# JiaxuanYou/graph-pooling

Measured on AMD Instinct MI355X. Metric: graphs/sec fwd+bwd, DD padded batch N_max=500, higher is better.
Workload: dtype f32; 1 GPU; S-DD: DD-shaped padded batch, B=20/GPU, N_max=500, F=89, H=E=20, K=50, L=3, 1 pool; graphs_per_gpu=20, global_batch=20, linkpred=False, hip_graph=True, parallelism=dp1

## Files before the change

graph_pooling_amd/csrc/dp_common.h:

```cpp
#pragma once
#include <hip/hip_runtime.h>
#include <cstddef>
#include <cstdint>
#include <cstdio>
#include <cstring>
#include <atomic>
#include <mutex>

#include "../../include/diffpool_hip.h"

namespace dp {

void set_error(const char* fmt, ...);
const char* last_error();

#define DP_CHECK_ARG(cond, ...)                      \
    do {                                             \
        if (!(cond)) {                               \
            ::dp::set_error(__VA_ARGS__);            \
            return DP_ERR_INVALID_ARG;               \
        }                                            \
    } while (0)

int* device_error_word();
// ... 449 lines not shown
    const float* stats[DP_MAX_LAYERS];
    const float* Z[2];
    int ldz[2];
    int coff[2][DP_MAX_LAYERS];
    int K;
    long wp_off, bp_off;
    const float* S;
    const float* Tt;
    const float* dXn;
    const float* dAn;
    const float* d_assign;
    const float* dZe;
    const unsigned short *pkA, *pkAt;
    int pk_ld;
    const int* pk_flag;
    const int* pk_sym;
    float* slabs;
    long slab_gstride;
    unsigned short* vs;
    float* part;
    float* gpart;
    int* bar;
};
bool level0_bwd_persistent_ok(const Level0Bwd& a);
size_t level0_bwd_vs_elems(const Level0Bwd& a);
size_t level0_bwd_gpart_floats(const Level0Bwd& a);
void level0_backward(Seq& q, const Level0Bwd& a);
bool level0_persistent_ok(const Level0Fwd& a);
size_t level0_bar_ints(int B);
int* level0_seq_word(int* bar);
size_t level0_xpart_floats(const Level0Fwd& a);
size_t level0_vs_elems(const Level0Fwd& a);
size_t level0_part_floats(const Level0Fwd& a);
size_t level0_mpart_floats(const Level0Fwd& a);
const int* level0_error_word(const int* bar);
void level0_forward(Seq& q, const Level0Fwd& a);

struct HeadArgs {
    const float* Z;
    int ldz, n, rw, featoff;
    int* argmax;
    int lda;
    const float* params;
    int n_pred;
    int dims[DP_MAX_PRED + 2];
    long w_off[DP_MAX_PRED + 1], b_off[DP_MAX_PRED + 1];
    float* hid[DP_MAX_PRED + 2];
    int B;
    long long* labels;
    const int* poison[DP_MAX_LEVELS + 1];
    int n_poison;
};
struct HeadBwdArgs {
    HeadArgs h;
    const float* d_ypred;
    float* grads;
    int n_levels;
    struct Level {
        float* dZ;
        const int* argmax;
        int lda, n, ldz, rw, featoff;
    } lv[DP_MAX_LEVELS + 1];
};
bool head_supported(const HeadArgs& a);
void head_fwd(Seq& q, const HeadArgs& a);
void head_bwd(Seq& q, const HeadBwdArgs& a);

bool small_level_fused_ok(int B, int n, const int* dims, int L, bool dadj);
size_t small_level_part_floats(int B, int n, int L);
void small_level_fwd(Seq& q, const SmallLevelIO& io, int B, int n, const int* dims, int L, int add_self, int bn);
struct SmallHeadFold {
    HeadBwdArgs hb;
    int level;
    int zcol;
    float* part;
};
size_t small_head_fold_part_floats(const HeadArgs& h);
long head_grad_entries(const HeadArgs& h);
void reduce_slabs_head(Seq& q, const float* slabs, long stride, int B, float* out, long count,
                       const SmallHeadFold& hf);
bool small_head_fold_fits(int B, int n, const int* dims, int L, bool dadj, const HeadArgs& h);
void small_level_bwd(Seq& q, const SmallLevelIO& io, const float* dZe, float* dX0, float* dadj, float* slabs,
                     long slab_stride, int B, int n, const int* dims, int L, int add_self, int bn,
                     const SmallHeadFold* hf = nullptr);

void build_batch(Seq& q, const int* src, const int* dst, const int* edge_ptr, const int* label, const int* node_ptr,
                 float* adj, unsigned short* pk, unsigned short* pkt, float* feats, float* assign, int* num_nodes,
                 int* errors, int* degree, int B, int N, int F, int mode, int symmetric, int max_edges_per_graph);

void gather_labels(Seq& q, const long long* src, long long* dst, int B);

void clip_adam_step(Seq& q, float* params, float* grads, float* exp_avg, float* exp_avg_sq, long n, float max_norm,
                    float beta1, float beta2, float eps, float step_size, float inv_bc2_sqrt, float* total_norm_out,
                    int* step_counter = nullptr, float lr = 0.f);

void csr_aggregate_fwd(Seq& q, const float* table, int ldt, const int* indptr, const int* indices, float* out, int ldo,
                       int n_rows, int feat, int mean, float beta, const float* values = nullptr);
void csr_aggregate_bwd_scatter(Seq& q, const float* dout, int ldo, const int* indptr, const int* indices, float* dtable,
                               int ldt, int n_rows, int feat, int mean, const float* values = nullptr);

void segment_max_part(Seq& q, const float* Z, int ldz, const int* chunk_tab, int n_chunks, int F, float* pv, int* pi);

void set2set_prep_weights(Seq& q, const float* w_ih, const float* w_hh, float* wt, int d);

struct LinkPlan {
    int kt, cw;
    int col_tiles, splits, split_tiles;
    int fwd_tiles;
    size_t fwd_lds, bwd_lds;
};
bool linkpred_plan(int B, int n, int K, LinkPlan& p);
void linkpred_fwd(Seq& q, const float* S, int lds, const float* adj, const int* num_nodes, float* loss_out,
                  int B, int n, int K, const float* norm = nullptr );
void linkpred_bwd(Seq& q, const float* S, int lds, const float* adj, const int* num_nodes, const float* dloss,
                  float* dS, int ldds, int B, int n, int K, int accumulate, const float* norm = nullptr);
void linkpred_fwd_packed(Seq& q, const float* S, int lds, const unsigned short* pk, const int* num_nodes,
                         float* loss_out, int B, int n, int K, const float* norm = nullptr);
void linkpred_bwd_packed(Seq& q, const float* S, int lds, const unsigned short* pk, const unsigned short* pkt,
                         const int* num_nodes, const float* dloss, float* dS, int ldds, int B, int n, int K,
                         int accumulate, const float* norm = nullptr);

struct AssignEntPick {
    int lanes;
    int quad;
};
AssignEntPick assign_ent_pick(const void* S, int lds, const void* dS, int ldds, int K);
size_t assign_ent_part_doubles();
void assign_entropy_fwd(Seq& q, const float* S, int lds, const int* num_nodes, float weight, float* ent_out,
                        float* total_inout, int B, int n, int K);
void assign_entropy_bwd(Seq& q, const float* S, int lds, const int* num_nodes, const float* dloss, float weight,
                        float* dS, int ldds, int accumulate, int B, int n, int K);

size_t frob_link_ws_doubles(long long rows, int B, int K);
void frob_link_w_dense(Seq& q, const float* S, int lds, const void* adj, const void* adj_t, int packed, int ld,
                       const int* num_nodes, float* W, int B, int N, int K);
void frob_link_fwd(Seq& q, const float* S, int lds, const float* W, const void* adj, int adj_kind, int adj_ld,
                   const int* num_nodes, const int* node_off, const int* nnz_ptr, const float* link_norm, float wscale,
                   float* G, float* loss_out, float* total_inout, int B, int N, long long rows, int K,
                   const int* csr_indptr = nullptr );
void frob_link_bwd(Seq& q, const float* S, int lds, const float* W, const float* G, const int* num_nodes,
                   const int* node_off, const float* link_norm, const float* dloss, float wscale, float* dS, int ldds,
                   int accumulate, int B, int N, long long rows, int K);

}
```

graph_pooling_amd/csrc/dp_level0.hip:

```cpp
#include "dp_common.h"
#include <type_traits>
#include <utility>
#include <vector>

namespace dp {

#ifdef DP_STAMP
__device__ unsigned long long g_l0_stamps[3][64];
#define L0_STAMP(i)                                                                                    \
    do {                                                                                               \
        if (threadIdx.x == 0 && (wid == 0 || wid == (int)gridDim.x / 2 || wid == (int)gridDim.x - 1)) \
            g_l0_stamps[wid == 0 ? 0 : (wid == (int)gridDim.x - 1 ? 2 : 1)][i] = __builtin_amdgcn_s_memtime(); \
    } while (0)
#else
#define L0_STAMP(i) \
    do {            \
    } while (0)
#endif

namespace {

typedef float f32x4 __attribute__((ext_vector_type(4)));
typedef float f32x4_u __attribute__((ext_vector_type(4), aligned(4)));
typedef short s16x8 __attribute__((ext_vector_type(8)));
// ... 111 lines not shown
        int* pollw = a.f.bar + BAR_GRAPH0 + b * BAR_GSTRIDE;
        const int target = ep.graph * a.T + a.target_bias;
        if (ok) {
            int it = 0;
            while (ag_ld(pollw) < target) {
                if (++it > a.spin_limit) {
                    ok = 0;
                    ag_st(a.f.bar + BAR_ERR, 1);
                    dev_err_raise(a.dev_err, DP_DEVERR_BARRIER);
                    break;
                }
                __builtin_amdgcn_s_sleep(1);
            }
        }
        sflag[0] = ok;
        if (!ok) sflag[1] = 1;
    }
    __syncthreads();
    return sflag[0] != 0;
}
template <typename Args>
__device__ inline bool l0_barrier(const Args& a, int b, int* sflag, L0Epoch& ep) {
    l0_arrive(a, b, sflag, ep);
    return l0_wait(a, b, sflag, ep);
}

template <int NI, typename Args>
__device__ __forceinline__ bool l0_poll_entries(const Args& a, ScBuf buf, const unsigned (&off)[NI], int B, unsigned tag,
                                                float (&v0)[NI][L0_BPAIRS], float (&v1)[NI][L0_BPAIRS], int* sflag) {
    const int tl = threadIdx.x & 15;
    const unsigned want = tag ^ (a.target_bias ? 0x40000000u : 0u);
    int it = 0;
    for (;;) {
        bool ready = true;
#pragma unroll
        for (int j = 0; j < NI; ++j) {
#pragma unroll
            for (int u = 0; u < L0_BPAIRS; ++u) {
                if (16 * u < B) {
                    const u32x4 q = sc_ld16(buf, off[j] + 16u * (unsigned)min(tl + 16 * u, B - 1));
                    v0[j][u] = __uint_as_float(q[0]);
                    v1[j][u] = __uint_as_float(q[2]);
                    ready = ready && q[1] == want && q[3] == want;
                } else {
                    v0[j][u] = 0.f;
                    v1[j][u] = 0.f;
                }
            }
        }
        if (__all(ready)) return true;
        if (++it > a.spin_limit || sflag[1]) {
            if (!sflag[1]) {
                sflag[1] = 1;
                ag_st(a.f.bar + BAR_ERR, 1);
                dev_err_raise(a.dev_err, DP_DEVERR_BARRIER);
            }
            return false;
        }
        __builtin_amdgcn_s_sleep(2);
    }
}

template <int QN>
__device__ __forceinline__ void l0_copy_in(float* dst, const float* src, int count, int zero_to = 0) {
    const int nq = count >> 2;
    float tail = 0.f;
    const int te = (nq << 2) + (int)threadIdx.x;
    if (te < count) tail = src[te];
    for (int base = 0; base < nq; base += QN * L0_NT) {
        f32x4_u q[QN];
#pragma unroll
        for (int u = 0; u < QN; ++u)
            q[u] = *reinterpret_cast<const f32x4_u*>(src + 4 * min(base + u * L0_NT + (int)threadIdx.x, nq - 1));
#pragma unroll
        for (int u = 0; u < QN; ++u) {
            const int e4 = base + u * L0_NT + (int)threadIdx.x;
            if (e4 < nq) *reinterpret_cast<f32x4*>(dst + 4 * e4) = q[u];
        }
    }
    if (te < count) dst[te] = tail;
    for (int e = count + (int)threadIdx.x; e < zero_to; e += L0_NT) dst[e] = 0.f;
}

template <int QN>
struct L0CopyStage {
    f32x4_u q[QN];
    float tail;
};
template <int QN>
__device__ __forceinline__ void l0_copy_issue(L0CopyStage<QN>& s, const float* src, int count, const void* safe) {
    const int nq = count >> 2;
    s.tail = src[min((nq << 2) + (int)threadIdx.x, count - 1)];
    const float* const qs = nq > 0 ? src : static_cast<const float*>(safe);
#pragma unroll
    for (int u = 0; u < QN; ++u)
        s.q[u] = *reinterpret_cast<const f32x4_u*>(qs + 4 * min(u * L0_NT + (int)threadIdx.x, max(nq - 1, 0)));
}
template <int QN>
__device__ __forceinline__ void l0_copy_commit(const L0CopyStage<QN>& s, float* dst, int count, int zero_to = 0) {
    const int nq = count >> 2;
    const int te = (nq << 2) + (int)threadIdx.x;
#pragma unroll
    for (int u = 0; u < QN; ++u) {
        const int e4 = u * L0_NT + (int)threadIdx.x;
        if (e4 < nq) *reinterpret_cast<f32x4*>(dst + 4 * e4) = s.q[u];
    }
    if (te < count) dst[te] = s.tail;
    for (int e = count + (int)threadIdx.x; e < zero_to; e += L0_NT) dst[e] = 0.f;
}
template <int QN>
__device__ __forceinline__ void l0_copy_rest(float* dst, const float* src, int count) {
    const int nq = count >> 2;
#pragma unroll 1
    for (int e4 = QN * L0_NT + (int)threadIdx.x; e4 < nq; e4 += L0_NT)
        *reinterpret_cast<f32x4*>(dst + 4 * e4) = *reinterpret_cast<const f32x4_u*>(src + 4 * e4);
}

__device__ inline void l0_write_split(ScBuf vsb, const float* PT, int ct, int CTt, int K8, int k8_0, int nk8, int nrows) {
    const long pl = (long)CTt * K8 * 128;
    const int items = nk8 * CTt * 16;
    for (int item = threadIdx.x; item < items; item += L0_NT) {
        const int c = item & 15, t = item >> 4;
        const int k8l = t / CTt, cb = t - k8l * CTt;
        const int vc = cb * 16 + c, lr = k8l * 8;
        u16x8 h, m, l;
#pragma unroll
        for (int j = 0; j < 8; ++j) {
            const float v = (vc < ct && lr + j < nrows) ? PT[(lr + j) * ct + min(vc, ct - 1)] : 0.f;
            unsigned short hh, mm, ll;
            bf16_split3(v, hh, mm, ll);
            h[j] = hh; m[j] = mm; l[j] = ll;
        }
        const long o = vs_index(0, CTt, K8, cb, k8_0 + k8l, c, 0);
        sc_st16(vsb, (unsigned)(o * 2), __builtin_bit_cast(u32x4, h));
        sc_st16(vsb, (unsigned)((o + pl) * 2), __builtin_bit_cast(u32x4, m));
        sc_st16(vsb, (unsigned)((o + 2 * pl) * 2), __builtin_bit_cast(u32x4, l));
    }
}

template <int MI, int CTH>
__device__ __forceinline__ void l0_agg_bf16(const unsigned short* Alds, int ldp, const unsigned short* vsp, int CTt, int K8,
                                            int steps, int rot, int cb0, f32x4 (&acc)[MI][CTH]) {
    int lane = threadIdx.x & 63;
    asm volatile("" : "+v"(lane));
    const int kh = __builtin_amdgcn_readfirstlane(threadIdx.x >> 6) & 3;
    const int l15 = lane & 15, kq = lane >> 4;
    auto eff = [&](int step) {
        const int s2 = min(step, steps - 1) + rot;
        return s2 >= steps ? s2 - steps : s2;
    };
    auto load_b = [&](int step, s16x8 (&dst)[3][CTH]) {
        const int st = eff(step);
#pragma unroll
        for (int p = 0; p < 3; ++p)
#pragma unroll
            for (int cbi = 0; cbi < CTH; ++cbi) {
                const int cb = min(cb0 + cbi, CTt - 1);
                const long o = ((((long)p * CTt + cb) * K8 + st * 4 + kq) * 16 + l15) * 8;
                dst[p][cbi] = *reinterpret_cast<const s16x8*>(vsp + o);
            }
    };
    auto mma = [&](int step, const s16x8 (&bf)[3][CTH]) {
        s16x8 av[MI];
#pragma unroll
        for (int rb = 0; rb < MI; ++rb)
            av[rb] = *reinterpret_cast<const s16x8*>(Alds + (rb * 16 + l15) * ldp + eff(step) * 32 + kq * 8);
// ... 279 lines not shown
                const int c = seg * 512 + 4 * tq;
                if (seg > 0) {
#pragma unroll
                    for (int u = 0; u < 4 * MI; ++u)
                        v[u] = *reinterpret_cast<const f32x4_u*>(Ab + (long)min(tr + 4 * u, nrows - 1) * N + min(c, N - 4));
                }
#pragma unroll
                for (int u = 0; u < 4 * MI; ++u) {
                    const int row = tr + 4 * u;
                    const bool in = row < nrows && c < N;
                    u16x4 h;
#pragma unroll
                    for (int j = 0; j < 4; ++j) {
                        const unsigned bits = in ? __float_as_uint(v[u][j]) : 0u;
                        bad |= (bits & 0xFFFFu) != 0;
                        h[j] = (unsigned short)(bits >> 16);
                    }
                    if (c < a.ldp) *reinterpret_cast<u16x4*>(Alds + row * a.ldp + c) = h;
                    if (row < nrows && c < f.pk_ld) *reinterpret_cast<u16x4*>(Pb + (long)row * f.pk_ld + c) = h;
                }
            }
        } else {
            for (int seg = 0; seg < segs; ++seg) {
                if (seg > 0) l0_stage_issue<MI>(q, Pb, f.pk_ld, nrows, seg);
                l0_stage_commit<MI>(q, Alds, a.ldp, f.pk_ld, nrows, seg);
            }
        }
    };
    if (f.A) phase0(std::true_type{});
    else phase0(std::false_type{});
    L0_STAMP(5);
    if (f.zero_p) {
        uint4* zp = reinterpret_cast<uint4*>(f.zero_p);
        const long nwg = gridDim.x, per = (a.zero_n16 + nwg - 1) / nwg;
        const long end = min(a.zero_n16, ((long)wid + 1) * per);
        for (long i = (long)wid * per + tid; i < end; i += L0_NT) zp[i] = make_uint4(0, 0, 0, 0);
    }
    if (__any(bad) && lane == 0) sflag[2] = 1;
    lds_barrier();
    const bool blk_bad = sflag[2] != 0;
    if (blk_bad && tid == 0) {
        ag_st(f.bar + BAR_GRAPH0 + b * BAR_GSTRIDE + BAR_G_INEXACT, 1);
        ag_st(f.bar + BAR_GFLAG, 1);
    }
    if (f.A) {
        const ScBuf atb = sc_buf(f.pkAt + (long)b * N * f.pk_ld, (size_t)N * f.pk_ld * 2);
        constexpr int P8 = RB / 8;
        for (int e = tid; e < N * P8; e += L0_NT) {
            const int k = e / P8, i8 = e - k * P8;
            if (r0 + i8 * 8 < f.pk_ld) {
                u16x8 h;
#pragma unroll
                for (int j = 0; j < 8; ++j) h[j] = Alds[(i8 * 8 + j) * a.ldp + k];
                sc_st16(atb, (unsigned)(((long)k * f.pk_ld + r0 + i8 * 8) * 2), __builtin_bit_cast(u32x4, h));
            }
        }
    }
    int ct = ct0;
    for (int slot = __builtin_amdgcn_readfirstlane(tid >> 6); slot <= 2 * L; slot += L0_NW) {
        float v0 = 0.f;
        if (slot < 2 * L) {
            const int l = slot >> 1, g = slot & 1;
            if (g < G && f.st[g].b_off[l] >= 0 && lane < f.st[g].dims[l + 1]) v0 = f.params[f.st[g].b_off[l] + lane];
        } else if (G == 2 && f.bp_off >= 0 && lane < f.K) {
            v0 = f.params[f.bp_off + lane];
        }
        BIAS[(slot < 2 * L ? slot : 2 * DP_MAX_LAYERS) * 64 + lane] = v0;
    }
    L0_STAMP(6);
    bool ok = l0_barrier(a, b, sflag, ep);
    L0_STAMP(7);
    const bool exact = !f.A || ag_ld(f.bar + BAR_GRAPH0 + b * BAR_GSTRIDE + BAR_G_INEXACT) == 0;
    const float* Arows = f.A + ((long)b * N + r0) * N;
    const float* Acols = f.A + (long)b * N * N + r0;

    constexpr int ITEMS = (RB * 2 + L0_TEAMS - 1) / L0_TEAMS;
    for (int l = 0; l < L; ++l) {
        const bool last = l == L - 1;
        const int w0 = f.st[0].dims[l + 1], w1 = G == 2 ? f.st[1].dims[l + 1] : 0;
        const int wmax = max(w0, w1);
        const int CTt = (ct + 15) / 16;
        const int ctp = CTt * 16 + 1;
        float* red = SCR;
        l0_aggregate<MI>(a, Alds, exact, Arows, N, 1, nrows, vs_rd(l, CTt), CTt, red, ctp, rot);
        L0_STAMP(8 + 8 * l);
        int wn0 = 0, wn1 = 0;
        float* const Wn0 = red + 4 * RB * ctp;
        if (!last) {
            wn0 = f.st[0].dims[l + 1] * f.st[0].dims[l + 2];
            wn1 = G == 2 ? f.st[1].dims[l + 1] * f.st[1].dims[l + 2] : 0;
        }
        float* const Wn1 = Wn0 + ((wn0 + 3) & ~3);
        if (!last) {
            l0_copy_in<4>(Wn0, f.params + f.st[0].w_off[l + 1], wn0);
            if (G == 2) l0_copy_in<4>(Wn1, f.params + f.st[1].w_off[l + 1], wn1);
        }
        lds_barrier();
        L0_STAMP(9 + 8 * l);
        const ScBuf partw = sc_buf(f.part + (long)l * f.B * N * G * 4, (size_t)f.B * N * G * 4 * sizeof(float));
        const unsigned bn_tag = (seq << 4) | (unsigned)(l + 1);
#pragma unroll
        for (int j = 0; j < ITEMS; ++j) {
            float yv[L0_NK];
            const int it = team + j * L0_TEAMS;
            const int r = min(G == 2 ? it >> 1 : it, RB - 1), g = G == 2 ? (it & 1) : 0;
            const bool on = it < RB * G && r < nrows;
            const long row = (long)b * N + min(r0 + r, N - 1);
            const int wg = g ? w1 : w0, c0gg = g ? w0 : 0;
            const float* bias = BIAS + (2 * l + g) * 64;
            float ss = 0.f;
#pragma unroll
            for (int k = 0; k < L0_NK; ++k) {
                yv[k] = 0.f;
                if (16 * k < wmax) {
                    const int c = min(tl + 16 * k, wg - 1);
                    const int o = r * ctp + c0gg + c;
                    float v = ((red[o] + red[RB * ctp + o]) + (red[2 * RB * ctp + o] + red[3 * RB * ctp + o])) + bias[c];
                    v = tl + 16 * k < wg ? v : 0.f;
                    yv[k] = v;
                    ss += v * v;
                }
            }
            ss = row16_sum(ss);
            const float inv = ss > L0_L2_EPS * L0_L2_EPS ? __builtin_amdgcn_rsqf(ss) : 1.f / L0_L2_EPS;
            float s1 = 0.f;
            float* yg = last ? f.Z[g] + row * f.ldz[g] + f.coff[g][l] : f.Y[l] + row * ct + c0gg;
            float* act = (g ? ACT1 : ACT0) + r * f.ldz[g] + f.coff[g][l];
#pragma unroll
            for (int k = 0; k < L0_NK; ++k) {
                if (16 * k < wmax) {
                    const int c = tl + 16 * k;
                    yv[k] *= inv;
                    if (on && c < wg) yg[c] = yv[k];
                    if (it < RB * G && c < wg) act[c] = r < nrows ? yv[k] : 0.f;
                    s1 += fmaxf(yv[k], 0.f);
                }
            }
            if (on && tl == 0) f.invn[l][row * G + g] = inv;
            if (!last && f.bn) {
                s1 = row16_sum(s1);
                const float mean = s1 / (float)wg;
                float m2 = 0.f;
#pragma unroll
                for (int k = 0; k < L0_NK; ++k) {
                    if (16 * k < wmax) {
                        const float v = (tl + 16 * k < wg) ? fmaxf(yv[k], 0.f) - mean : 0.f;
                        m2 += v * v;
                    }
                }
                m2 = row16_sum(m2);
                if (on && tl == 0) {
                    const long po = (((long)min(r0 + r, N - 1) * G + g) * f.B + b) * 16;
                    sc_st16(partw, (unsigned)po, sc_tagged(mean, m2, bn_tag));
                }
            }
        }
        L0_STAMP(10 + 8 * l);
        if (last) break;
        if (!f.bn) lds_barrier();
        L0_STAMP(11 + 8 * l);
        const int ctn = f.st[0].dims[l + 2] + (G == 2 ? f.st[1].dims[l + 2] : 0);
        float* PTn = Wn1 + ((wn1 + 3) & ~3);
        {
            float pm[ITEMS][L0_BPAIRS], pq[ITEMS][L0_BPAIRS];
            if (f.bn) {
                unsigned off[ITEMS];
#pragma unroll
                for (int j = 0; j < ITEMS; ++j) {
                    const int it = team + j * L0_TEAMS;
                    const int r = min(G == 2 ? it >> 1 : it, RB - 1), g = G == 2 ? (it & 1) : 0;
                    off[j] = (unsigned)((((long)min(r0 + r, N - 1) * G + g) * f.B) * 16);
                }
                ok = l0_poll_entries<ITEMS>(a, partw, off, f.B, bn_tag, pm, pq, sflag) && ok;
            }
#pragma unroll
            for (int j = 0; j < ITEMS; ++j) {
                const int it = team + j * L0_TEAMS;
                const int r = min(G == 2 ? it >> 1 : it, RB - 1), g = G == 2 ? (it & 1) : 0;
                const bool on = it < RB * G && r < nrows;
// ... 1256 lines not shown
```

graph_pooling_amd/csrc/dp_model.hip:

```cpp
#include "dp_common.h"

namespace dp {

void set2set_fwd(Seq& q, const float* emb, int lde, const float* w_ih, const float* w_hh, const float* b_ih,
                 const float* b_hh, const float* Wp, const float* bp, float* out, int B, int n, int d, void* save);
void set2set_bwd(Seq& q, const float* emb, int lde, const float* w_ih, const float* w_hh, const float* b_ih,
                 const float* b_hh, const float* Wp, const float* bp, const float* out, const float* dout,
                 float* demb, int ldde, float* dw_ih, float* dw_hh, float* db_ih, float* db_hh, float* dWp,
                 float* dbp, int B, int n, int d, const void* save);
size_t set2set_save_bytes(int B, int n, int d);

namespace {

struct LevelInfo {
    int j;
    int n, G, L;
    const dp_stack_cfg* e;
    const dp_stack_cfg* a;
    int D, Da, K;
    int ctot[DP_MAX_LAYERS];
    int coff_e[DP_MAX_LAYERS], coff_a[DP_MAX_LAYERS];
    int cmax;
};

// ... 433 lines not shown
            gather_cols(q, lv.Ze + li.coff_e[l - 1], li.D, de, li.a ? lv.Za + li.coff_a[l - 1] : nullptr, li.Da, da, Pj,
                        (long)B * n);
            aggregate(q, io.adj, Pj, cin, Uin, cin, B, n, cin, false, 0.f, pk, vs, false);
            if (add_self) axpy(q, Uin, Pj, 1.f, (long)B * n * cin);
            const int dins[2] = {de, da}, c0ins[2] = {0, de};
            widen_fused = last && widen_fwd_supported(groups_of(li, l), dins);
            if (!widen_fused) {
                GemmDesc d[2];
                for (int gi = 0; gi < li.G; ++gi) {
                    const dp_stack_cfg* st = gi == 0 ? li.e : li.a;
                    const int c0 = gi == 0 ? 0 : li.e->dims[l + 1], c0in = gi == 0 ? 0 : de;
                    d[gi] = GemmDesc{Uin + c0in, PW(params, st->w_off[l]), Pj + c0, nullptr, n, st->dims[l + 1],
                                     st->dims[l], cin, st->dims[l + 1], ct, (long)n * cin, 0, (long)n * ct, false, false,
                                     1.f, 0.f, 0};
                }
                bgemm_group(q, d, li.G, B);
            } else {
                const float* Wg[2] = {PW(params, li.e->w_off[l]), li.a ? PW(params, li.a->w_off[l]) : nullptr};
                widen_fwd(q, Uin, cin, c0ins, dins, Wg, layer_bias(li, params, l), groups_of(li, l),
                          concat_slice<GroupPtrs>(li, l, lv.Ze, lv.Za), lv.layer[l].invn, (long)B * n, 1);
            }
        } else if (!transformed) {
            transform(q, B, li, lv, io, params, l, Pj, presplit ? vs : nullptr);
        }
        transformed = false;
        if (l == 0 && io.pack) {
            const bool folded = q.fold_zero_p == nullptr;
            q.fold_zero_p = nullptr;
            q.fold_zero_n16 = 0;
            adj_pack(q, io.pack->adj, io.pack->pkA, io.pack->pkAt, io.pack->flag, B, n, io.pack->ld, folded,
                     io.pack->zero_p, io.pack->zero_bytes);
        }
        RowGroups g = groups_of(li, l);
        const GroupCPtrs bias = layer_bias(li, params, l);
        const GroupPtrs xout = concat_slice<GroupPtrs>(li, l, lv.Ze, lv.Za);
        const GroupPtrs yout = last ? xout : layer_y<GroupPtrs>(li, lv, l);
        const int stats_mode = (!last && bn) ? 1 : 0;
        if (widen_fused) {
        } else if (agg_first) {
            rownorm_fwd(q, Pj, ct, nullptr, bias, g, yout, lv.layer[l].invn, stats_mode ? part : nullptr, (long)B * n, 1,
                        stats_mode);
        } else if (!aggregate_rownorm_fwd(q, io.adj, Pj, ct, add_self ? Pj : nullptr, bias, g, yout, lv.layer[l].invn,
                                   stats_mode ? part : nullptr, B, n, 1, stats_mode, pk, vs, presplit)) {
            aggregate(q, io.adj, Pj, ct, Uj, ct, B, n, ct, false, 0.f, pk, vs, presplit);
            rownorm_fwd(q, Uj, ct, add_self ? Pj : nullptr, bias, g, yout, lv.layer[l].invn,
                        stats_mode ? part : nullptr, (long)B * n, 1, stats_mode);
        }
        if (!last) {
            const RowGroups gnext = groups_of(li, l + 1);
            const float* part_r = bn ? bn_exchange(q, p, part, sc.part_all, (size_t)B * n * li.G * 2) : nullptr;
            bool plain_next = !p.sync_bn && !knobs().no_level_fusion && bn_transform_supported(g, gnext, B) &&
                              !layer_agg_first(li, l + 1);
            for (int gi = 0; gi < li.G; ++gi) plain_next = plain_next && !drop_mask(li, io, gi, l + 1);
            if (plain_next) {
                const float* Wn[2] = {PW(params, li.e->w_off[l + 1]), li.a ? PW(params, li.a->w_off[l + 1]) : nullptr};
                const int ctn = li.ctot[l + 1];
                const bool presplit_n = pk && vs && aggregate_packed_usable(io.adj, n, ctn);
                bn_transform_fwd(q, lv.layer[l].Y, ct, bn ? part : nullptr, lv.layer[l].stats, g, xout, Wn, gnext, Pj,
                                 ctn, B, n, 1, presplit_n ? vs : nullptr);
                transformed = true;
            } else {
                bn_apply_fwd(q, lv.layer[l].Y, ct, part_r, lv.layer[l].stats, g, xout, B, n, 1, B * W);
            }
        }
    }
}

void level_backward(Seq& q, const EncoderPlan& p, int j, const LevelSave& lv, const LevelIO& io, const float* params,
                    const Scratch& sc) {
    const dp_encoder_cfg& c = *p.c;
    const LevelInfo& li = p.lv[j];
    const LevelGrad& gr = *io.gr;
    const int B = c.B, n = li.n;
    const int W = bn_world(c);
    float *const slabs = sc.slabs, *const Pj = sc.Pj, *const dUj = sc.Uj, *const Gj = sc.Gj, *const part = sc.part;
    const long slab_stride = sc.slab_stride;
    const long gstride = slab_stride * sc.KS;
    const int ks_level = n >= 256 ? sc.KS : 1;
    const PackedAdj* const pk = io.pk;
    unsigned short* const vs = sc.vs;
    const bool bn = c.flags & DP_F_BN;
    const bool add_self = c.flags & DP_F_ADD_SELF;
    if (p.bwd[j] == Tier::WholeLevel) {
        small_level_bwd(q, small_level_io(li, lv, io, params, sc.lvl_part), gr.dZe, gr.dX0, gr.dAdj, slabs, gstride, B,
                        n, li.e->dims, li.L, add_self ? 1 : 0, bn ? 1 : 0, io.hf);
        return;
    }
    if (p.bwd[j] == Tier::PerLayer) {
        float* pbuf[2] = {part, sc.part_b};
        for (int l = li.L - 1; l >= 0; --l) {
            const bool last = l == li.L - 1;
            const bool has_bn = !last && bn;
            const int din = li.e->dims[l], dout = li.e->dims[l + 1];
            const float* xin = l == 0 ? io.x0e : lv.Ze + li.coff_e[l - 1];
            const int ldxin = l == 0 ? din : li.D;
            float* dxin = l > 0 ? gr.dZe + li.coff_e[l - 1] : gr.dX0;
            const int lddxin = l > 0 ? li.D : din;
            small_gcn_bwd(q, io.adj, xin, ldxin, PW(params, li.e->w_off[l]),
                          last ? lv.Ze + li.coff_e[l] : lv.layer[l].Y, last ? li.D : li.ctot[l],
                          has_bn ? lv.Ze + li.coff_e[l] : nullptr, li.D, lv.layer[l].invn, lv.layer[l].stats,
                          has_bn ? pbuf[l & 1] : nullptr, gr.dZe + li.coff_e[l], li.D, dxin, lddxin,
                          (l > 0 && bn && dxin) ? pbuf[(l - 1) & 1] : nullptr, gr.dAdj, slabs + li.e->w_off[l],
                          li.e->b_off[l] >= 0 ? slabs + li.e->b_off[l] : nullptr, gstride, B, n, din, dout,
                          add_self ? 1 : 0, has_bn ? 1 : 0, last ? 0 : 1);
        }
        return;
    }
    bool part_ready = false;
    for (int l = li.L - 1; l >= 0; --l) {
        const int ct = li.ctot[l];
        const bool last = l == li.L - 1;
        RowGroups g = groups_of(li, l);
        const GroupCPtrs dx = concat_slice<GroupCPtrs>(li, l, gr.dZe, gr.dZa);
        const GroupCPtrs xhat = concat_slice<GroupCPtrs>(li, l, lv.Ze, lv.Za);
        const GroupCPtrs y = last ? xhat : layer_y<GroupCPtrs>(li, lv, l);
        const bool has_bn = !last && bn;
        const float* part2 = part;
        if (has_bn) {
            if (!part_ready) bn_bwd_partials(q, dx, xhat, g, part, (long)B * n);
            part2 = bn_exchange(q, p, part, sc.part_all, (size_t)B * n * li.G * 2);
        }
        part_ready = false;
        GroupPtrs dbias{};
        dbias.p[0] = li.e->b_off[l] >= 0 ? slabs + li.e->b_off[l] : nullptr;
        dbias.p[1] = (li.a && li.a->b_off[l] >= 0) ? slabs + li.a->b_off[l] : nullptr;
        dbias.ld[0] = dbias.ld[1] = (int)gstride;
        const bool agg_first = layer_agg_first(li, l) && !gr.dAdj;
        const bool presplit = !agg_first && pk && vs && aggregate_packed_usable(io.adj, n, ct);
        bool mv_fused = false;
        if (agg_first) {
            const int dins[2] = {li.e->dims[l], li.a ? li.a->dims[l] : 0}, c0ins[2] = {0, li.e->dims[l]};
            mv_fused = rownorm_bwd_mv_supported(g, dins, n);
            if (mv_fused) {
                const float* Wg[2] = {PW(params, li.e->w_off[l]), li.a ? PW(params, li.a->w_off[l]) : nullptr};
                rownorm_bwd_mv(q, dx, xhat, y, lv.layer[l].invn, lv.layer[l].stats, part2, g, dUj, ct, &dbias, B, n,
                               !last, has_bn, 1, B * W, Wg, dins, c0ins, Gj, layer_cin(li, l));
            }
        }
        if (!mv_fused)
            rownorm_bwd(q, dx, xhat, y, lv.layer[l].invn, lv.layer[l].stats, part2, g, dUj, ct, &dbias, B, n, !last,
                        has_bn, 1, presplit ? vs : nullptr, B * W);
        if (agg_first) {
            const int cin = layer_cin(li, l), de = li.e->dims[l], da = li.a ? li.a->dims[l] : 0;
            const float* Uin = lv.layer[l].Uin;
            GemmDesc d[4];
            int nd = 0;
            for (int gi = 0; gi < li.G; ++gi) {
                const dp_stack_cfg* st = gi == 0 ? li.e : li.a;
                const int din = st->dims[l], dout = st->dims[l + 1], c0in = gi == 0 ? 0 : de;
                d[nd++] = GemmDesc{Uin + c0in, dUj + g.c0[gi], slabs + st->w_off[l], nullptr, din, dout, n, cin, ct, dout,
                                   (long)n * cin, (long)n * ct, gstride, true, false, 1.f, 0.f, 0, slab_stride, 0};
                if (!mv_fused)
                    d[nd++] = GemmDesc{dUj + g.c0[gi], PW(params, st->w_off[l]), Gj + c0in, nullptr, n, din, dout, ct,
                                       dout, cin, (long)n * ct, 0, (long)n * cin, false, true, 1.f, 0.f, 0, 0, 0, nullptr,
                                       0, 0, 0, 1};
            }
            bgemm_group(q, d, nd, B, ks_level);
            float* dxagg = dUj;
            aggregate(q, io.adj, Gj, cin, dxagg, cin, B, n, cin, true, 0.f, pk, vs, false);
            if (add_self) axpy(q, dxagg, Gj, 1.f, (long)B * n * cin);
            if (bn && !knobs().no_rowpart_hook && scatter_add_cols_part_supported(de, da)) {
                scatter_add_cols_part(q, dxagg, concat_slice<GroupPtrs>(li, l - 1, gr.dZe, gr.dZa),
                                      concat_slice<GroupCPtrs>(li, l - 1, lv.Ze, lv.Za), de, da, li.G, part, (long)B * n);
                part_ready = true;
            } else {
                scatter_add_cols(q, dxagg, gr.dZe + li.coff_e[l - 1], li.D, de,
                                 li.a ? gr.dZa + li.coff_a[l - 1] : nullptr, li.Da, da, (long)B * n);
            }
// ... 655 lines not shown
```

graph_pooling_amd/csrc/dp_small.hip:

```cpp
#include "dp_common.h"

namespace dp {

#define SM_L2_EPS 1e-12f
#define SM_BN_EPS 1e-5f

#ifdef DP_STAMP
__device__ unsigned long long g_small_stamps[2][32];
#define SM_STAMP(k, i)                                                                       \
    do {                                                                                     \
        if (blockIdx.x == 0 && threadIdx.x == 0) g_small_stamps[k][i] = __builtin_amdgcn_s_memtime(); \
    } while (0)
#else
#define SM_STAMP(k, i) \
    do {               \
    } while (0)
#endif

namespace {

__device__ inline float sm_team_sum(float v) {
    return row16_sum(v);
}

// ... 533 lines not shown
                }
                m2 = sm_team_sum(m2);
                if (tl == 0) sc_st16(part_l, (unsigned)(((long)r * a.B + b) * 16), sc_tagged(mean, m2, (seq << 4) | (unsigned)(l + 1)));
            }
        }
        SM_STAMP(0, 12 + 6 * l);
        if (last) break;
        if (stats) {
            SM_STAMP(0, 13 + 6 * l);
            for (int r = team; r < n; r += NTEAMS) {
                float pm[SM_BMAX16], pq[SM_BMAX16];
                const bool ok = sm_poll_row(part_l, (unsigned)((long)r * a.B * 16), a.B, bn_tag, pm, pq, a.spin_limit, a.bar,
                                            a.dev_err);
                float sm = 0.f;
#pragma unroll
                for (int u = 0; u < SM_BMAX16; ++u) sm += (tl + 16 * u < a.B) ? pm[u] : 0.f;
                float m = sm_team_sum(sm) / (float)a.B;
                float s2 = 0.f;
#pragma unroll
                for (int u = 0; u < SM_BMAX16; ++u) {
                    const float d = pm[u] - m;
                    s2 += (tl + 16 * u < a.B) ? pq[u] + (float)dout * d * d : 0.f;
                }
                float rstd = 1.0f / sqrtf(sm_team_sum(s2) / ((float)a.B * (float)dout) + SM_BN_EPS);
                if (!ok) m = rstd = __builtin_nanf("");
                if (tl == 0) {
                    if (b == 0) {
                        a.stats[l][r * 2] = m;
                        a.stats[l][r * 2 + 1] = rstd;
                    }
                    mu[r] = m;
                    rs[r] = rstd;
                }
            }
            SM_STAMP(0, 14 + 6 * l);
        } else {
            for (int r = tid; r < n; r += NT) {
                mu[r] = 0.f;
                rs[r] = 1.f;
            }
        }
        lds_barrier();
        for (int r = team; r < n; r += NTEAMS)
            for (int k = tl; k < dout; k += 16) {
                const float v = (fmaxf(U[r * dout + k], 0.f) - mu[r]) * rs[r];
                X[r * dout + k] = v;
                a.Ze[((long)b * n + r) * a.ldz + a.coff[l] + k] = v;
            }
        lds_barrier();
        SM_STAMP(0, 15 + 6 * l);
        wo += din * dout;
        bo += dout;
    }
    sm_finish(a.bar, a.seq, seq, a.B);
}

struct SmallLevelBwdArgs {
    const float* adj;
    const float* x0;
    int ldx0;
    const float* params;
    long w_off[DP_MAX_LAYERS], b_off[DP_MAX_LAYERS];
    int dims[DP_MAX_LAYERS + 1];
    int L;
    const float* Y[DP_MAX_LAYERS];
    int ldY[DP_MAX_LAYERS];
    const float* invn[DP_MAX_LAYERS];
    const float* stats[DP_MAX_LAYERS];
    const float* Ze;
    int ldz;
    int coff[DP_MAX_LAYERS];
    const float* dZe;
    float* dX0;
    float* dadj;
    float* slabs;
    long slab_stride;
    float* part;
    int* bar;
    int* seq;
    int* dev_err;
    int spin_limit, target_bias;
    int B, n, add_self, bn;
    int omax, wtot, D;
    SmDiv qd0, qD;
    SmDiv qdout[DP_MAX_LAYERS];
    int fold, hlevel, zcol;
    HeadBwdArgs hb;
    float* hgrad;
};

struct SmHead {
    int nP, d0, d1, C, wup, hup;
    __host__ __device__ SmHead(const HeadArgs& h) : nP(h.n_pred), d0(h.dims[0]), d1(h.dims[1]), C(h.dims[h.n_pred]) {
        wup = hup = 0;
        for (int i = 1; i < nP; ++i) {
            wup += h.dims[i] * h.dims[i + 1];
            hup += h.dims[i];
        }
    }
    __host__ __device__ size_t lds_floats() const { return (size_t)d1 * d0 + wup + 2 * (size_t)hup + (size_t)C; }
};

__global__ __launch_bounds__(1024) void k_small_level_bwd(SmallLevelBwdArgs a) {
    extern __shared__ __attribute__((aligned(16))) float lds[];
    const int b = blockIdx.x, tid = threadIdx.x;
    const int n = a.n, L = a.L, D = a.D, d0 = a.dims[0];
    const unsigned seq = (unsigned)a.seq[0];
    float* A = lds;
    float* DA = A + n * n;
    float* X0 = DA + (a.dadj ? n * n : 0);
    float* ZE = X0 + n * d0;
    float* DZ = ZE + n * D;
    float* YS = DZ + n * D;
    float* WL = YS + (L - 1) * n * a.omax;
    float* IV = WL + a.wtot;
    float* RS = IV + L * n;
    float* dU = RS + L * n;
    float* G = dU + n * a.omax;
    float* P = G + n * a.omax;
    float* M0 = P + n * a.omax;
    float* M1 = M0 + n;
    float* DB = M1 + n;
    float* DBW = DB + a.omax;
    const int tl = tid & 15, team = tid >> 4;
    const int NT = blockDim.x, NTEAMS = blockDim.x >> 4;
    const SmHead hz(a.hb.h);
    float* HW0 = DBW + 16 * a.omax;
    float* HWU = HW0 + hz.d1 * hz.d0;
    float* HH = HWU + hz.wup;
    float* HG = HH + hz.hup;
    float* HY = HG + hz.hup;
    SM_STAMP(1, 16);
    int win = -1;
    if (a.fold) {
        if (tid < hz.d0) {
            for (int lv = 0; lv < a.hb.n_levels; ++lv) {
                const int f = tid - a.hb.lv[lv].featoff;
                if (f >= 0 && f < a.hb.lv[lv].rw) win = a.hb.lv[lv].argmax[(long)b * a.hb.lv[lv].lda + f];
            }
        }
        const HeadArgs& h = a.hb.h;
        sm_dma(HY, hz.C, [&](int e) { return a.hb.d_ypred + (long)b * hz.C + e; });
        sm_dma(HW0, hz.d1 * hz.d0, [&](int e) { return h.params + h.w_off[0] + e; });
        int wo = 0, ho = 0;
        for (int i = 1; i < hz.nP; ++i) {
            const int cnt = h.dims[i] * h.dims[i + 1];
            sm_dma(HWU + wo, cnt, [&](int e) { return h.params + h.w_off[i] + e; });
            sm_dma(HH + ho, h.dims[i], [&](int e) { return h.hid[i] + (long)b * h.dims[i] + e; });
            wo += cnt;
            ho += h.dims[i];
        }
    }

    sm_dma(A, n * n, [&](int e) { return a.adj + (long)b * n * n + e; });
    sm_dma(X0, n * d0, [&](int e) { return a.x0 + ((long)b * n + a.qd0.quot(e)) * a.ldx0 + a.qd0.rem(e); });
    sm_dma(ZE, n * D, [&](int e) { return a.Ze + ((long)b * n + a.qD.quot(e)) * a.ldz + a.qD.rem(e); });
    sm_dma(DZ, n * D, [&](int e) { return a.dZe + ((long)b * n + a.qD.quot(e)) * a.ldz + a.qD.rem(e); });
    {
        int wo = 0;
        for (int l = 0; l < L; ++l) {
            const int din = a.dims[l], dout = a.dims[l + 1];
            const float* w = a.params + a.w_off[l];
            sm_dma(WL + wo, din * dout, [&](int e) { return w + e; });
            wo += din * dout;
            const float* iv = a.invn[l] + (long)b * n;
            sm_dma(IV + l * n, n, [&](int e) { return iv + e; });
            if (l < L - 1) {
                const float* y = a.Y[l];
                const int ldy = a.ldY[l];
                const SmDiv q = a.qdout[l];
                sm_dma(YS + l * n * a.omax, n * dout, [&](int e) { return y + ((long)b * n + q.quot(e)) * ldy + q.rem(e); });
                if (a.bn) {
                    const float* st = a.stats[l];
                    sm_dma(RS + l * n, n, [&](int e) { return st + e * 2 + 1; });
                }
            }
        }
    }
    if (a.dadj)
        for (int i = tid; i < n * n; i += NT) DA[i] = 0.f;
    SM_STAMP(1, 17);
    __syncthreads();
    SM_STAMP(1, 18);

    if (a.fold) {
        const HeadArgs& h = a.hb.h;
        int ho = hz.hup, wo = hz.wup;
        for (int i = hz.nP - 1; i >= 1; --i) {
            const int din = h.dims[i], dout = h.dims[i + 1];
            wo -= din * dout;
            ho -= din;
            const float* go = i == hz.nP - 1 ? HY : HG + ho + din;
            const float* W = HWU + wo;
            for (int k = tid; k < din; k += NT) {
                float s = 0.f;
#pragma unroll 8
                for (int j = 0; j < dout; ++j) s += go[j] * W[j * din + k];
                HG[ho + k] = HH[ho + k] > 0.f ? s : 0.f;
            }
            __syncthreads();
        }
        for (int e = tid; e < hz.hup; e += NT) a.hgrad[(long)b * hz.hup + e] = HG[e];
        const float* g1 = hz.nP == 1 ? HY : HG;
        for (int k = tid, it = 0; k < hz.d0; k += NT, ++it) {
            float s = 0.f;
#pragma unroll 8
            for (int j = 0; j < hz.d1; ++j) s += g1[j] * HW0[j * hz.d0 + k];
            for (int lv = 0; lv < a.hb.n_levels; ++lv) {
                const HeadBwdArgs::Level& t = a.hb.lv[lv];
                const int f = k - t.featoff;
                if (f >= 0 && f < t.rw) {
                    const int r = it == 0 ? win : t.argmax[(long)b * t.lda + f];
                    if (r < 0) continue;
                    if (lv == a.hlevel) DZ[r * D + a.zcol + f] += s;
                    else t.dZ[((long)b * t.n + r) * t.ldz + f] = s;
                }
            }
        }
        SM_STAMP(1, 19);
    }

    int wo_end = a.wtot;
    for (int l = L - 1; l >= 0; --l) {
        const int din = a.dims[l], dout = a.dims[l + 1];
        const bool last = l == L - 1;
        const bool has_bn = !last && a.bn;
        const bool has_relu = !last;
        wo_end -= din * dout;
        const float* W = WL + wo_end;
        const float* Xl = l == 0 ? X0 : ZE + a.coff[l - 1];
        const int ldx = l == 0 ? d0 : D;
        const float* Yl = last ? ZE + a.coff[l] : YS + l * n * a.omax;
        const int ldy = last ? D : dout;
        float* dx = DZ + a.coff[l];
        for (int i = tid; i < 16 * dout; i += NT) DBW[i] = 0.f;
        if (has_bn) {
            const ScBuf part_l = sc_buf(a.part + (long)l * a.B * n * 4, (size_t)a.B * n * 16);
            const unsigned bn_tag = (seq << 4) | (unsigned)(l + 1);
            const float* xh = ZE + a.coff[l];
            for (int r = team; r < n; r += NTEAMS) {
                float s0 = 0.f, s1 = 0.f;
                for (int c = tl; c < dout; c += 16) {
                    const float d = dx[r * D + c];
                    s0 += d;
                    s1 += d * xh[r * D + c];
                }
                s0 = sm_team_sum(s0);
                s1 = sm_team_sum(s1);
                if (tl == 0) sc_st16(part_l, (unsigned)(((long)r * a.B + b) * 16), sc_tagged(s0, s1, bn_tag));
            }
            for (int r = team; r < n; r += NTEAMS) {
                float p0[SM_BMAX16], p1[SM_BMAX16];
                const bool ok = sm_poll_row(part_l, (unsigned)((long)r * a.B * 16), a.B,
                                            bn_tag ^ (a.target_bias ? 0x40000000u : 0u), p0, p1, a.spin_limit, a.bar, a.dev_err);
                float s0 = 0.f, s1 = 0.f;
#pragma unroll
                for (int u = 0; u < SM_BMAX16; ++u) {
                    s0 += (tl + 16 * u < a.B) ? p0[u] : 0.f;
                    s1 += (tl + 16 * u < a.B) ? p1[u] : 0.f;
                }
                s0 = sm_team_sum(s0);
                s1 = sm_team_sum(s1);
                const float cnt = (float)a.B * (float)dout;
// ... 164 lines not shown
        v = hipGetDeviceProperties(&prop, dev) == hipSuccess ? prop.multiProcessorCount : -1;
        cus[dev].store(v, std::memory_order_relaxed);
    }
    return v > 0 ? v : 0;
}
static bool level_kernels_admitted() {
    static std::atomic<int> state[64];
    int dev = 0;
    if (hipGetDevice(&dev) != hipSuccess || dev < 0 || dev >= 64) return false;
    int v = state[dev].load(std::memory_order_relaxed);
    if (v == 0) {
        v = 1;
        const void* fns[2] = {reinterpret_cast<const void*>(&k_small_level_fwd),
                              reinterpret_cast<const void*>(&k_small_level_bwd)};
        for (const void* fn : fns) {
            int blocks = 0;
            hipError_t e = hipFuncSetAttribute(fn, hipFuncAttributeMaxDynamicSharedMemorySize, 159 * 1024);
            if (e == hipSuccess) e = hipOccupancyMaxActiveBlocksPerMultiprocessor(&blocks, fn, 1024, 150 * 1024);
            if (e != hipSuccess || blocks < 1) {
                (void)hipGetLastError();
                set_error("whole-level kernels disabled: the runtime admits %d resident 1024-thread workgroups with 150 KiB "
                          "of LDS per CU (%s)", blocks, hipGetErrorString(e));
                v = -1;
            }
        }
        state[dev].store(v, std::memory_order_relaxed);
    }
    return v > 0;
}
bool small_level_fused_ok(int B, int n, const int* dims, int L, bool dadj) {
    if (knobs().no_level_fusion || L < 2 || L > DP_MAX_LAYERS || n > 64) return false;
    for (int l = 0; l <= L; ++l)
        if (dims[l] > 256 || (l > 0 && dims[l] > 64)) return false;
    if (small_level_lds_fwd(B, n, dims, L) * sizeof(float) > 150 * 1024) return false;
    if (small_level_lds_bwd(B, n, dims, L, dadj) * sizeof(float) > 150 * 1024) return false;
    const int cus = device_cus();
    return cus > 0 && B <= cus / 2 && B <= 16 * SM_BMAX16 && level_kernels_admitted();
}
size_t small_level_part_floats(int B, int n, int L) { return (size_t)(L > 1 ? L - 1 : 1) * B * n * 4; }
long head_grad_entries(const HeadArgs& h) {
    long tot = 0;
    for (int i = 0; i < h.n_pred; ++i) tot += (long)h.dims[i + 1] * (h.dims[i] + (h.b_off[i] >= 0 ? 1 : 0));
    return tot;
}
size_t small_head_fold_part_floats(const HeadArgs& h) {
    const SmHead z(h);
    return (size_t)h.B * (z.hup > 0 ? z.hup : 1);
}
bool small_head_fold_fits(int B, int n, const int* dims, int L, bool dadj, const HeadArgs& h) {
    if (h.n_pred < 1 || h.B != B || head_grad_entries(h) >= (1L << 30)) return false;
    return (small_level_lds_bwd(B, n, dims, L, dadj) + SmHead(h).lds_floats()) * sizeof(float) <= 150 * 1024;
}

void small_level_fwd(Seq& q, const SmallLevelIO& io, int B, int n, const int* dims, int L, int add_self, int bn) {
    if (!q.ok()) return;
    static DynLdsOnce attr;
    ensure_dyn_lds(q, attr, reinterpret_cast<const void*>(&k_small_level_fwd), 159 * 1024, "k_small_level_fwd");
    if (!q.ok()) return;
    SmallLevelFwdArgs a{};
    a.adj = io.adj; a.x0 = io.x0; a.ldx0 = io.ldx0; a.params = io.params; a.L = L;
    a.Ze = io.Ze; a.ldz = io.ldz; a.part = io.part; a.bar = io.bar; a.seq = q.seq_word;
    a.B = B; a.n = n; a.add_self = add_self; a.bn = bn;
    for (int l = 0; l <= L; ++l) a.dims[l] = dims[l];
    for (int l = 0; l < L; ++l) {
        a.w_off[l] = io.w_off[l]; a.b_off[l] = io.b_off[l];
        a.Y[l] = io.Y[l]; a.ldY[l] = io.ldY[l]; a.invn[l] = io.invn[l]; a.stats[l] = io.stats[l];
        a.coff[l] = io.coff[l];
        a.dmax = dims[l] > a.dmax ? dims[l] : a.dmax;
        a.omax = dims[l + 1] > a.omax ? dims[l + 1] : a.omax;
        a.wtot += dims[l] * dims[l + 1];
        a.btot += dims[l + 1];
    }
    a.qd0 = sm_div(dims[0]);
    a.dev_err = device_error_word();
    a.spin_limit = knobs().test_barrier_fail ? 64 : SM_SPIN_LIMIT;
    a.target_bias = knobs().test_barrier_fail ? 1 : 0;
    hipLaunchKernelGGL(k_small_level_fwd, dim3(B), dim3(1024), small_level_lds_fwd(B, n, dims, L) * sizeof(float),
                       q.stream, a);
    q.check_launch("small_level_fwd");
}

void small_level_bwd(Seq& q, const SmallLevelIO& io, const float* dZe, float* dX0, float* dadj, float* slabs,
                     long slab_stride, int B, int n, const int* dims, int L, int add_self, int bn,
                     const SmallHeadFold* hf) {
    if (!q.ok()) return;
    static DynLdsOnce attr;
    ensure_dyn_lds(q, attr, reinterpret_cast<const void*>(&k_small_level_bwd), 159 * 1024, "k_small_level_bwd");
    if (!q.ok()) return;
    SmallLevelBwdArgs a{};
    a.adj = io.adj; a.x0 = io.x0; a.ldx0 = io.ldx0; a.params = io.params; a.L = L;
    a.Ze = io.Ze; a.ldz = io.ldz; a.part = io.part; a.bar = io.bar; a.seq = q.seq_word;
    a.dZe = dZe; a.dX0 = dX0; a.dadj = dadj; a.slabs = slabs; a.slab_stride = slab_stride;
    a.B = B; a.n = n; a.add_self = add_self; a.bn = bn;
    for (int l = 0; l <= L; ++l) a.dims[l] = dims[l];
    for (int l = 0; l < L; ++l) {
        a.w_off[l] = io.w_off[l]; a.b_off[l] = io.b_off[l];
        a.Y[l] = io.Y[l]; a.ldY[l] = io.ldY[l]; a.invn[l] = io.invn[l]; a.stats[l] = io.stats[l];
        a.coff[l] = io.coff[l];
        a.omax = dims[l + 1] > a.omax ? dims[l + 1] : a.omax;
        a.wtot += dims[l] * dims[l + 1];
        a.D += dims[l + 1];
        a.qdout[l] = sm_div(dims[l + 1]);
    }
    a.qd0 = sm_div(dims[0]);
    a.qD = sm_div(a.D);
    a.dev_err = device_error_word();
    a.spin_limit = knobs().test_barrier_fail ? 64 : SM_SPIN_LIMIT;
    a.target_bias = knobs().test_barrier_fail ? 1 : 0;
    size_t lds = small_level_lds_bwd(B, n, dims, L, dadj != nullptr);
    if (hf) {
        a.fold = 1;
        a.hb = hf->hb;
        a.hlevel = hf->level;
        a.zcol = hf->zcol;
        a.hgrad = hf->part;
        lds += SmHead(hf->hb.h).lds_floats();
    }
    hipLaunchKernelGGL(k_small_level_bwd, dim3(B), dim3(1024), lds * sizeof(float), q.stream, a);
    q.check_launch("small_level_bwd");
}

#ifdef DP_STAMP
extern "C" __attribute__((visibility("default"))) int dp_debug_stamps(unsigned long long* out) {
    return (int)hipMemcpyFromSymbol(out, HIP_SYMBOL(g_small_stamps), sizeof(unsigned long long) * 64);
}
#endif

}
```

Measured before the change: 87330 graphs/s.

## Overlap next-layer weight DMA with aggregation; skip loading known-zero dZe

In the level-0 kernel, next-layer weights are now loaded straight into LDS with global_load_lds_dword, issued before the adjacency aggregation, so the copy runs during that compute instead of after it. A single vmcnt wait is placed before the barrier. Separately, the small-level backward kernel skips the global read of dZe when the caller flags it as all zeros (the last pooled level with head fold) and clears the LDS buffer instead. The first part relies on inline asm that manipulates m0 and on correct wave partitioning of the copy. The second assumes that dZe really is zero in that case.

```diff
diff --git a/graph_pooling_amd/csrc/dp_common.h b/graph_pooling_amd/csrc/dp_common.h
--- a/graph_pooling_amd/csrc/dp_common.h
+++ b/graph_pooling_amd/csrc/dp_common.h
@@ -555,7 +555,7 @@
 bool small_head_fold_fits(int B, int n, const int* dims, int L, bool dadj, const HeadArgs& h);
 void small_level_bwd(Seq& q, const SmallLevelIO& io, const float* dZe, float* dX0, float* dadj, float* slabs,
                      long slab_stride, int B, int n, const int* dims, int L, int add_self, int bn,
-                     const SmallHeadFold* hf = nullptr);
+                     const SmallHeadFold* hf = nullptr, bool dZe_zero = false);
 
 void build_batch(Seq& q, const int* src, const int* dst, const int* edge_ptr, const int* label, const int* node_ptr,
                  float* adj, unsigned short* pk, unsigned short* pkt, float* feats, float* assign, int* num_nodes,
diff --git a/graph_pooling_amd/csrc/dp_level0.hip b/graph_pooling_amd/csrc/dp_level0.hip
--- a/graph_pooling_amd/csrc/dp_level0.hip
+++ b/graph_pooling_amd/csrc/dp_level0.hip
@@ -217,6 +217,23 @@
     for (int e = count + (int)threadIdx.x; e < zero_to; e += L0_NT) dst[e] = 0.f;
 }
 
+__device__ __forceinline__ void l0_dma_in(float* dst, const float* src, int count, int first_wave = 0) {
+    const int lane = threadIdx.x & 63;
+    const int wave = (__builtin_amdgcn_readfirstlane(threadIdx.x >> 6) - first_wave) & (L0_NW - 1);
+    const unsigned base = (unsigned)(size_t)(__attribute__((address_space(3))) float*)dst;
+    for (int c0 = wave * 64; c0 < count; c0 += L0_NT) {
+        if (c0 + lane < count) {
+            const float* g = src + c0 + lane;
+            const unsigned piece = __builtin_amdgcn_readfirstlane(base + 4u * (unsigned)c0);
+            unsigned keep;
+            asm volatile("s_mov_b32 %0, m0\n\ts_mov_b32 m0, %2\n\ts_nop 0\n\tglobal_load_lds_dword %1, off\n\ts_mov_b32 m0, %0"
+                         : "=&s"(keep)
+                         : "v"(g), "s"(piece)
+                         : "memory");
+        }
+    }
+}
+
 template <int QN>
 struct L0CopyStage {
     f32x4_u q[QN];
@@ -662,8 +679,6 @@
         const int CTt = (ct + 15) / 16;
         const int ctp = CTt * 16 + 1;
         float* red = SCR;
-        l0_aggregate<MI>(a, Alds, exact, Arows, N, 1, nrows, vs_rd(l, CTt), CTt, red, ctp, rot);
-        L0_STAMP(8 + 8 * l);
         int wn0 = 0, wn1 = 0;
         float* const Wn0 = red + 4 * RB * ctp;
         if (!last) {
@@ -672,9 +687,12 @@
         }
         float* const Wn1 = Wn0 + ((wn0 + 3) & ~3);
         if (!last) {
-            l0_copy_in<4>(Wn0, f.params + f.st[0].w_off[l + 1], wn0);
-            if (G == 2) l0_copy_in<4>(Wn1, f.params + f.st[1].w_off[l + 1], wn1);
-        }
+            l0_dma_in(Wn0, f.params + f.st[0].w_off[l + 1], wn0);
+            if (G == 2) l0_dma_in(Wn1, f.params + f.st[1].w_off[l + 1], wn1, (wn0 + 63) >> 6);
+        }
+        l0_aggregate<MI>(a, Alds, exact, Arows, N, 1, nrows, vs_rd(l, CTt), CTt, red, ctp, rot);
+        L0_STAMP(8 + 8 * l);
+        asm volatile("s_waitcnt vmcnt(0)" ::: "memory");
         lds_barrier();
         L0_STAMP(9 + 8 * l);
         const ScBuf partw = sc_buf(f.part + (long)l * f.B * N * G * 4, (size_t)f.B * N * G * 4 * sizeof(float));
diff --git a/graph_pooling_amd/csrc/dp_model.hip b/graph_pooling_amd/csrc/dp_model.hip
--- a/graph_pooling_amd/csrc/dp_model.hip
+++ b/graph_pooling_amd/csrc/dp_model.hip
@@ -539,8 +539,9 @@
     const bool bn = c.flags & DP_F_BN;
     const bool add_self = c.flags & DP_F_ADD_SELF;
     if (p.bwd[j] == Tier::WholeLevel) {
+        const bool dZe_zero = io.hf != nullptr && j == c.num_pooling;
         small_level_bwd(q, small_level_io(li, lv, io, params, sc.lvl_part), gr.dZe, gr.dX0, gr.dAdj, slabs, gstride, B,
-                        n, li.e->dims, li.L, add_self ? 1 : 0, bn ? 1 : 0, io.hf);
+                        n, li.e->dims, li.L, add_self ? 1 : 0, bn ? 1 : 0, io.hf, dZe_zero);
         return;
     }
     if (p.bwd[j] == Tier::PerLayer) {
diff --git a/graph_pooling_amd/csrc/dp_small.hip b/graph_pooling_amd/csrc/dp_small.hip
--- a/graph_pooling_amd/csrc/dp_small.hip
+++ b/graph_pooling_amd/csrc/dp_small.hip
@@ -639,6 +639,7 @@
     int spin_limit, target_bias;
     int B, n, add_self, bn;
     int omax, wtot, D;
+    int dz_zero;
     SmDiv qd0, qD;
     SmDiv qdout[DP_MAX_LAYERS];
     int fold, hlevel, zcol;
@@ -712,7 +713,8 @@
     sm_dma(A, n * n, [&](int e) { return a.adj + (long)b * n * n + e; });
     sm_dma(X0, n * d0, [&](int e) { return a.x0 + ((long)b * n + a.qd0.quot(e)) * a.ldx0 + a.qd0.rem(e); });
     sm_dma(ZE, n * D, [&](int e) { return a.Ze + ((long)b * n + a.qD.quot(e)) * a.ldz + a.qD.rem(e); });
-    sm_dma(DZ, n * D, [&](int e) { return a.dZe + ((long)b * n + a.qD.quot(e)) * a.ldz + a.qD.rem(e); });
+    if (!a.dz_zero)
+        sm_dma(DZ, n * D, [&](int e) { return a.dZe + ((long)b * n + a.qD.quot(e)) * a.ldz + a.qD.rem(e); });
     {
         int wo = 0;
         for (int l = 0; l < L; ++l) {
@@ -736,6 +738,8 @@
     }
     if (a.dadj)
         for (int i = tid; i < n * n; i += NT) DA[i] = 0.f;
+    if (a.dz_zero)
+        for (int i = tid; i < n * D; i += NT) DZ[i] = 0.f;
     SM_STAMP(1, 17);
     __syncthreads();
     SM_STAMP(1, 18);
@@ -1066,7 +1070,7 @@
 
 void small_level_bwd(Seq& q, const SmallLevelIO& io, const float* dZe, float* dX0, float* dadj, float* slabs,
                      long slab_stride, int B, int n, const int* dims, int L, int add_self, int bn,
-                     const SmallHeadFold* hf) {
+                     const SmallHeadFold* hf, bool dZe_zero) {
     if (!q.ok()) return;
     static DynLdsOnce attr;
     ensure_dyn_lds(q, attr, reinterpret_cast<const void*>(&k_small_level_bwd), 159 * 1024, "k_small_level_bwd");
@@ -1091,6 +1095,7 @@
     a.dev_err = device_error_word();
     a.spin_limit = knobs().test_barrier_fail ? 64 : SM_SPIN_LIMIT;
     a.target_bias = knobs().test_barrier_fail ? 1 : 0;
+    a.dz_zero = dZe_zero ? 1 : 0;
     size_t lds = small_level_lds_bwd(B, n, dims, L, dadj != nullptr);
     if (hf) {
         a.fold = 1;
```

Result: no change. 87940 graphs/s, median of 6 (+0.7%).
